# fjdf/slaMEM

Hardware: AMD Instinct MI355X
Metric: MEMs/sec (and queries/sec) on 100 Mbp ref x 10 M 150 bp queries, l=20 (higher is better)
Workload: dtype u32; 1 GPU; synthetic 100000000 bp reference (splitmix64 seed 42) x 10000000 reads/GPU of 150 bp, 2% substitutions, 50% reverse-complemented, -b -l 20; ref_len=100000000, reads_total=10000000, read_len=150, min_len=20, both_strands=True, parallelism=query shards x1, one GPU, no replication

## Files before the change

include/slamem_hip.h:

```cpp
#ifndef SLAMEM_HIP_H
#define SLAMEM_HIP_H

#include <stddef.h>
#include <stdint.h>

#ifdef __cplusplus
extern "C" {
#endif

#define SLAMEM_ABI_VERSION 4

enum {
    SLAMEM_OK = 0,
    SLAMEM_ERR_ARG = 1,
    SLAMEM_ERR_HIP = 2,
    SLAMEM_ERR_NOMEM = 3,
    SLAMEM_ERR_CAPACITY = 4,
    SLAMEM_ERR_FORMAT = 5,
    SLAMEM_ERR_IO = 6,
    SLAMEM_ERR_NO_DEVICE = 7
};

typedef struct slamem_index slamem_index;

// ... 87 lines not shown
    uint64_t skips;
    uint64_t enum_row_steps;
    uint64_t enum_levels;
    uint64_t enum_wave_us;
    uint64_t state_lane_trips[11];
    uint64_t state_wave_trips[11];
    uint64_t seed_windows;
    uint64_t seed_compares;
    uint64_t seed_letter_masks;
    uint64_t seed_mems;
    uint64_t seed_strands_left;
    uint64_t seed_reads;
    uint64_t seed_query_bytes;
    uint64_t seed_left_why[7];
    uint64_t seed_once_reads;
} slamem_search_stats;

int slamem_abi_version(void);
const char *slamem_strerror(int code);
const char *slamem_last_error_message(void);
int slamem_device_count(int *count_out);
int slamem_device_warmup(int device);
int slamem_device_pci_bus_id(int device, char *out, int out_bytes);
int slamem_device_mem_info(int device, uint64_t *free_out, uint64_t *total_out);
int slamem_get_timings(slamem_timings *out);
int slamem_reset_timings(void);
int slamem_search_stats_enable(int on);
int slamem_get_search_stats(slamem_search_stats *out);
int slamem_get_search_clock(double *us_to_empty_list, double *us_tail, double *us_wave_sum);

// ... 289 lines not shown
```

slamem_amd/capi.py:

```python
from __future__ import annotations

import ctypes as C
import os

_HERE = os.path.dirname(os.path.abspath(__file__))
LIB_PATH = os.environ.get("SLAMEM_HIP_LIB") or os.path.join(_HERE, "csrc", "libslamem_hip.so")
SYNTH_PATH = os.path.join(_HERE, "csrc", "libslamem_synth.so")

SLAMEM_OK = 0
SLAMEM_ERR_ARG = 1
SLAMEM_ERR_HIP = 2
SLAMEM_ERR_NOMEM = 3
SLAMEM_ERR_CAPACITY = 4
SLAMEM_ERR_FORMAT = 5
SLAMEM_ERR_IO = 6
SLAMEM_ERR_NO_DEVICE = 7

ARRAY_SA, ARRAY_BWT, ARRAY_LCP, ARRAY_PSV, ARRAY_NSV = range(5)
LAYOUT_AUTO, LAYOUT_FULL, LAYOUT_COMPACT = 0, 1, 2

ABI_SYMBOLS = (
    "slamem_abi_version", "slamem_strerror", "slamem_last_error_message", "slamem_device_count",
    "slamem_get_timings", "slamem_reset_timings", "slamem_device_warmup", "slamem_device_pci_bus_id",
    "slamem_index_build", "slamem_index_build_device", "slamem_index_build_layout", "slamem_index_build_device_layout",
# ... 62 lines not shown
                ("k8_ms_sum", C.c_double), ("seed_ms", C.c_float), ("mum_filter_ms", C.c_float), ("seed_ms_sum", C.c_double)]

    def as_dict(self):
        return {k: getattr(self, k) for k, _ in self._fields_}


class SearchStats(C.Structure):
    _fields_ = [(k, C.c_uint64) for k in (
        "fm_lines_top", "fm_lines_bottom", "rec_lines_fail", "rec_lines_pend", "rec_lines_flush", "query_loads",
        "lane_trips", "wave_trips", "positions", "enum_jobs", "prefilter_probes", "prefilter_query_loads",
        "prefilter_items", "items", "survivors", "mems", "overflow_records", "valid", "dir_sa_lines", "dir_group_loads",
        "dir_rec_lines", "dir_letters", "jump_lines", "skip_group_loads", "skip_probe_lines", "skip_attempts", "skips",
        "enum_row_steps", "enum_levels", "enum_wave_us")] + [("state_lane_trips", C.c_uint64 * 11),
                                                               ("state_wave_trips", C.c_uint64 * 11)] + [
        (k, C.c_uint64) for k in ("seed_windows", "seed_compares", "seed_letter_masks", "seed_mems", "seed_strands_left",
                                  "seed_reads", "seed_query_bytes")] + [("seed_left_why", C.c_uint64 * 7), ("seed_once_reads", C.c_uint64)]

    def as_dict(self):
        return {k: (list(getattr(self, k)) if (k.startswith("state_") or k == "seed_left_why") else int(getattr(self, k))) for k, _ in self._fields_}


_LIB = None
_SYNTH = None


class GtParams(C.Structure):
    _fields_ = [("ploidy", C.c_uint32), ("match_cost", C.c_uint32), ("het_cost", C.c_uint32), ("err_cost", C.c_uint32),
                ("het_prior", C.c_uint32), ("min_depth", C.c_uint32), ("min_qual", C.c_uint32)]


def _declare(L):
# ... 177 lines not shown
```

slamem_amd/csrc/mem_search.hip:

```cpp
#include "common.h"
#include "prims.h"

#include <atomic>
#include <type_traits>
#include <new>
#include <stdlib.h>
#include <string.h>

namespace slamem {

struct Blk {
    uint4 a;
    uint4 b;
    uint4 c;
    uint4 d;
};

__device__ __forceinline__ uint64_t u64_of(uint32_t lo, uint32_t hi) { return ((uint64_t)hi << 32) | lo; }

__device__ __forceinline__ Blk load_blk(const FMBlock* __restrict__ fm, uint32_t bi) {
    const uint4* p = reinterpret_cast<const uint4*>(fm + bi);
    Blk k;
    k.a = p[0]; k.b = p[1]; k.c = p[2]; k.d = p[3];
    return k;
// ... 120 lines not shown
    uint64_t num_items;
    uint8_t* item_attempt;
    const uint8_t* item_alive;
    const uint32_t* work_ids;
    const uint32_t* work_count;
    unsigned long long* stats;
    uint64_t query_words;
    const uint64_t* pq;
    uint64_t* pq_out;
    uint32_t implicit_items;
    uint32_t* seed_left_ids;
    unsigned int* seed_left_count;
    unsigned int* seed_long_flag;
    unsigned int* seed_wide;
    uint32_t seed_step;
    const uint64_t* item_pk;
    unsigned int* work_cursor;
    int32_t direct_min_depth;
    uint32_t use_jump;
    uint32_t pad2;
    uint32_t skip_w;
    const uint64_t* pq2;
    uint64_t* pq2_out;
    uint8_t* item_flags;
    uint32_t skip_s1;
    uint32_t pad4;
    const struct SliceState* slice_state;
    const uint32_t* item_block;
    struct OutCtx {
        struct RawRow* inline_rows;
// ... 806 lines not shown
        const uint2 e = A.defer.list[i];
        uint32_t* c = A.defer.pool + e.y;
        const uint32_t jobs = c[0], own = c[1];
        uint32_t run = 0;
        for (uint32_t s2 = 0; s2 < jobs; s2++) { const uint32_t v = c[2u + s2]; c[2u + s2] = run; run += v; }
        c[2u + jobs] = run;
        A.block_counts[e.x] = own + run;
    }
}

enum : uint32_t {
    SC_FM_TOP = 0, SC_FM_BOT, SC_REC_FAIL_LINES, SC_REC_PEND_LINES, SC_REC_FLUSH_LINES, SC_QUERY_LOADS, SC_LANE_TRIPS,
    SC_WAVE_TRIPS, SC_POSITIONS, SC_ENUM_JOBS, SC_ENUM_ROW_STEPS, SC_PF_PROBES, SC_PF_QUERY_LOADS, SC_PF_ITEMS,
    SC_DIR_SA, SC_DIR_GROUPS, SC_DIR_RECS, SC_DIR_QLOADS, SC_DIR_LETTERS, SC_JUMP_LINES,
    SC_SKIP_GROUPS, SC_SKIP_QLOADS, SC_SKIP_PROBES, SC_SKIP_OK, SC_T_FIRST, SC_T_DRAIN, SC_T_LAST, SC_T_WAVE_SUM, SC_ENUM_LEVELS, SC_T_ENUM_SUM, SC_STATE_TRIPS , SC_STATE_WAVES = SC_STATE_TRIPS + 11 ,
    SC_SEED_WINDOWS = SC_STATE_WAVES + 11, SC_SEED_COMPARES, SC_SEED_NMASKS, SC_SEED_MEMS, SC_SEED_LEFT, SC_SEED_READS, SC_SEED_QBYTES, SC_SEED_WHY , SC_SEED_ONCE = SC_SEED_WHY + 7, SC_COUNT
};
template <bool kStats>
__device__ __forceinline__ void stat_flush(unsigned long long* dst, uint32_t v) {
    if (!kStats) return;
    for (int o = 32; o > 0; o >>= 1) v += __shfl_down(v, o);
    if ((threadIdx.x & 63u) == 0u && v) atomicAdd(dst, (unsigned long long)v);
}

template <uint32_t kLanes>
__global__ void __launch_bounds__(256) k_pack_queries(SearchArgs A, bool long_only) {
    __shared__ uint8_t lut[512];
    for (uint32_t i = threadIdx.x; i < 256u; i += 256u) {
        uint32_t c = ascii_code_q(i);
        lut[i] = (uint8_t)c;
        lut[256u + i] = (uint8_t)(c >= 2u ? 7u - c : c);
// ... 1051 lines not shown
        const uint32_t g = list[i];
        const ItemDesc d = item_of(A, g);
        uint32_t n_probe = 0, n_qload = 0;
        if (!prefilter_item<false>(A, d, n_probe, n_qload)) alive[g] = 0;
    }
}

#ifndef SLAMEM_SEED_READS
#define SLAMEM_SEED_READS 21
#endif
constexpr uint32_t kSeedReads = SLAMEM_SEED_READS, kSeedReadsMid = 16, kSeedReadsLong = 16;
constexpr uint32_t kSeedMaxLen = 192;
constexpr uint32_t kSeedMaxLenMid = 256;
constexpr uint32_t kSeedMaxLenLong = 384;
#ifndef SLAMEM_SEED_JOBS
#define SLAMEM_SEED_JOBS 16
#endif
constexpr uint32_t kSeedJobs = SLAMEM_SEED_JOBS;
#ifndef SLAMEM_SEED_MEMS
#define SLAMEM_SEED_MEMS 12
#endif
constexpr uint32_t kSeedMems = SLAMEM_SEED_MEMS;
constexpr uint32_t kSigLetters = 12, kSigMask = (1u << kSigLetters) - 1u, kSigKnown = 1u << 24;

template <uint32_t NW, uint32_t R>
struct SeedWave {
    static constexpr uint32_t kJobs = kSeedJobs * R * NW / 3u, kMems = kSeedMems * R * NW / 3u;
    uint64_t pl[R][2][2][NW + 1];
    uint32_t len[R];
    uint32_t nwin[R];
    union {
        uint4 raw[R * NW * 4 + 1];
        struct {
            uint32_t job_p[kJobs], job_x[kJobs];
            uint32_t mem_key[kMems], mem_ref[kMems];
            uint32_t mem_sig[kMems];
        };
    };
    uint32_t bad[R];
    uint64_t pn[R][NW + 1];
    uint32_t hasn;
    unsigned long long expl[R];
    union {
        uint16_t ring[128];
        unsigned long long smask[2 * R];
    };
    uint32_t flags;
    uint32_t pad[3];
};

__device__ __forceinline__ void wave_sync() {
    __builtin_amdgcn_fence(__ATOMIC_RELEASE, "wavefront");
    __builtin_amdgcn_wave_barrier();
    __builtin_amdgcn_fence(__ATOMIC_ACQUIRE, "wavefront");
}
__device__ __forceinline__ uint64_t funnel64(uint64_t lo, uint64_t hi, uint32_t sh) { return (lo >> sh) | ((hi << 1) << (63u - sh)); }
__device__ __forceinline__ uint64_t bits_below(int x) {
    const int c = x < 0 ? 0 : x > 64 ? 64 : x;
    return c == 0 ? 0ull : (~0ull >> (64 - c));
}
__device__ __forceinline__ uint64_t bits_range(int lo, int hi) { return bits_below(hi) & ~bits_below(lo); }
__device__ __forceinline__ uint32_t sel4(const uint4& v, uint32_t a) {
    const uint32_t lo = (a & 1u) ? v.y : v.x, hi = (a & 1u) ? v.w : v.z;
    return (a & 2u) ? hi : lo;
// ... 2 lines not shown
    const uint32_t a = e & 3u, x0 = sel4(b0, a), x1 = sel4(b1, a), x2 = sel4(b2, a);
    return e < 4u ? x0 : e < 8u ? x1 : x2;
}
__device__ __forceinline__ uint32_t byte_tops(uint32_t m) {
    const uint32_t y = m >> 7;
    return (y | (y >> 7) | (y >> 14) | (y >> 21)) & 0xFu;
}

#ifndef SLAMEM_SEED_WAVES
#define SLAMEM_SEED_WAVES 1
#endif
template <bool kStats, uint32_t NW, uint32_t R>
__global__ void __launch_bounds__(256, SLAMEM_SEED_WAVES) k_seed_mems(SearchArgs A, uint8_t* __restrict__ alive) {
    constexpr uint32_t kMaxLen = 64u * NW;
    static_assert(R <= 32u && R * NW <= 128u, "a flag word holds a bit per read; the planes step runs in at most two passes");
    __shared__ SeedWave<NW, R> lds[4];
    const IndexView& ix = A.ix;
    const uint32_t lane = threadIdx.x & 63u, wv = threadIdx.x >> 6;
    SeedWave<NW, R>& S = lds[wv];
    const uint32_t strands = A.strands, k = ix.seed_k, L = A.min_len, s = L - k + 1u;
    const uint32_t kmask = (1u << k) - 1u;
    const uint64_t r0 = ((uint64_t)blockIdx.x * 4u + wv) * R;
    if (r0 >= (uint64_t)A.num_queries) return;
    const uint32_t nr = (uint64_t)A.num_queries - r0 < R ? (uint32_t)((uint64_t)A.num_queries - r0) : R;
    const unsigned long long below = (1ull << lane) - 1ull;
    const int64_t ulast = (int64_t)text_units(ix.n) - 1;
    uint32_t n_win = 0, n_cmp = 0, n_nm = 0, n_mem = 0;

    const uint64_t off = lane <= nr ? A.offsets[r0 + lane] : 0ull;
    constexpr uint32_t kRawChunks = R * NW * 4u + 1u, kSpecIters = (kRawChunks + 63u) / 64u;
// ... 142 lines not shown
                const uint64_t* f = S.pl[i][0][pl];
                const uint64_t lo = w + q < NW ? __brevll(f[NW - 1u - (w + q)]) : 0ull, hi = w + q + 1u < NW ? __brevll(f[NW - 2u - (w + q)]) : 0ull;
                S.pl[i][1][pl][w] = Li ? ~funnel64(lo, hi, r) & bits_range(0, (int)Li - 64 * (int)w) : 0ull;
            }
        }
    }
    {
        const bool isbad = lane < nr && plen != 0u && S.bad[lane] != 0u;
        wflags |= (uint32_t)__ballot(isbad);
        if (isbad) nwin = 0;
        if (lane < nr) { S.len[lane] = nwin ? len : 0u; S.nwin[lane] = nwin; }
    }
    if (lane == 0u)
        for (uint32_t i = nr; i < R; i++) { S.len[i] = 0u; S.nwin[i] = 0u; }
    wave_sync();
    const uint32_t mfit = k / s > 6u ? 6u : k / s;
    const uint32_t mstep = A.seed_step ? A.seed_step : mfit >= 3u ? mfit : s <= 12u ? 2u : 1u;

    const bool wave_hasn = __builtin_amdgcn_readfirstlane((int)S.hasn) != 0;
    uint32_t lg_slots = 0;
    {
        const uint32_t nwl = lane < nr ? S.nwin[lane] : 0u;
#pragma unroll
        for (uint32_t t = 1, lg = 1; t <= 32u; t <<= 1, lg++)
            if (__ballot(nwl > t) != 0ull) lg_slots = lg;
    }
    if (lane < R) S.expl[lane] = 0ull;
    uint32_t njobs = 0, nmems = 0;

    auto search = [&](auto with_n) {
    constexpr bool hasn = decltype(with_n)::value;
    auto trip = [&](uint32_t ent, bool act, uint32_t step) {
        const uint32_t rs = ent >> 8, wi = ent & 0xFFu;
        const uint32_t Lr = act ? S.len[rs] : 0u;
        const uint32_t o = wi * s;
        uint32_t want = 0, pal = 0;
        uint4 b0 = make_uint4(0, 0, 0, 0), b1 = b0, b2 = b0, b3 = b0;
        if (hasn && act) {
            const uint64_t* PN = S.pn[rs];
            if (((uint32_t)funnel64(PN[o >> 6], PN[(o >> 6) + 1u], o & 63u) & kmask) != 0u) act = false;
        }
        if (act) {
            const uint32_t q = o >> 6, sh = o & 63u;
            const uint64_t* P0 = S.pl[rs][0][0];
            const uint64_t* P1 = S.pl[rs][0][1];
            const uint32_t f0 = (uint32_t)funnel64(P0[q], P0[q + 1u], sh) & kmask, f1 = (uint32_t)funnel64(P1[q], P1[q + 1u], sh) & kmask;
            uint32_t bucket, tagbits, orient;
            seed_place(f0, f1, k, ix.seed_log2, bucket, tagbits, orient, pal);
            want = tagbits | (orient << 7);
            const uint4* B = reinterpret_cast<const uint4*>(ix.seed + bucket);
            b0 = B[0]; b1 = B[1]; b2 = B[2]; b3 = B[3];
        }
        if (kStats) n_win += (uint32_t)__popcll(__ballot(act));
        const uint32_t wbytes = want * 0x01010101u;
        const uint32_t x0 = b3.x ^ wbytes, x1 = b3.y ^ wbytes, x2 = b3.z ^ wbytes;
        const uint32_t m0 = ~((x0 & 0x7F7F7F7Fu) + 0x7F7F7F7Fu) & 0x80808080u, m1 = ~((x1 & 0x7F7F7F7Fu) + 0x7F7F7F7Fu) & 0x80808080u,
                       m2 = ~((x2 & 0x7F7F7F7Fu) + 0x7F7F7F7Fu) & 0x80808080u;
        const uint32_t count = b3.w;
        uint32_t hits = byte_tops(m0) | (byte_tops(m1) << 4) | (byte_tops(m2) << 8);
        const uint32_t rev = byte_tops(x0 & 0x80808080u) | (byte_tops(x1 & 0x80808080u) << 4) | (byte_tops(x2 & 0x80808080u) << 8);
        hits &= count >= kSeedSlots ? 0xFFFu : (1u << count) - 1u;
        if (strands == 1u && step == 1u) hits &= ~rev;
        if (!act) hits = 0;
        const uint32_t xn = act && (count & kSeedSpilled) ? (count >> 24) & 0x1Fu : 0u, xo = (count & 0xFFFFFFu) << 2;
        if (act && count > kSeedSlots && !(count & kSeedSpilled)) {
            atomicOr(&S.flags, 1u << rs);
            if (kStats) atomicAdd(A.stats + SC_SEED_WHY + 1u, 1ull);
            hits = 0;
        }
        const bool both = pal != 0u && strands == 2u;
        if (kStats && both && hits) atomicAdd(A.stats + SC_SEED_WHY + 2u, 1ull);
        const uint32_t e1 = hits ? (uint32_t)__ffs((int)hits) - 1u : 0u;
        const uint32_t p1 = sel12(b0, b1, b2, e1);
        const uint32_t st1 = (rev >> e1) & 1u;
        const uint32_t dist = step * s;
        uint32_t pn = 0, pp1 = 0, ps1 = 0;
        if (dist <= k) {
            pp1 = __shfl_up(p1, 1);
            ps1 = __shfl_up(hits ? st1 : 2u, 1);
            const uint32_t pent = __shfl_up(act ? ent : 0xFFFFFFFFu, 1);
            pn = (lane == 0u || wi < step || pent != ent - step || ps1 == 2u) ? 0u : 1u;
        }
        const uint32_t njobs0 = njobs;
        auto push = [&](bool hv, uint32_t p, uint32_t st) {
            const uint32_t w = st ? p + dist : p - dist;
            const bool job = hv && !(pn && pp1 == w && ps1 == st);
            const unsigned long long qb = __ballot(job);
            const uint32_t at = njobs + (uint32_t)__popcll(qb & below);
            if (job && at < SeedWave<NW, R>::kJobs) {
                S.job_p[at] = p;
                S.job_x[at] = (st ? Lr - k - o : o) | (st << 15) | (rs << 16);
            }
            njobs += (uint32_t)__popcll(qb);
        };
        uint32_t rem = hits;
        for (uint32_t it = 0; __ballot(rem != 0u) != 0ull; it++) {
            const bool hv = rem != 0u;
            const uint32_t e = it == 0u ? e1 : hv ? (uint32_t)__ffs((int)rem) - 1u : 0u;
            rem &= rem - 1u;
            const uint32_t p = it == 0u ? p1 : sel12(b0, b1, b2, e);
            push(hv, p, (rev >> e) & 1u);
            if (__ballot(hv && both) != 0ull) push(hv && both, p, 1u);
        }
        for (uint32_t e0 = 0; __ballot(e0 < xn) != 0ull; e0 += 4u) {
            const bool on = e0 < xn;
            uint4 v0 = make_uint4(0, 0, 0, 0), v1 = v0;
            if (on) {
                const uint4* P = reinterpret_cast<const uint4*>(ix.spill + xo + e0);
                v0 = P[0]; v1 = P[1];
            }
#pragma unroll
            for (uint32_t q = 0; q < 4u; q++) {
                const uint32_t p = q == 0u ? v0.x : q == 1u ? v0.z : q == 2u ? v1.x : v1.z;
                const uint32_t d = ((q == 0u ? v0.y : q == 1u ? v0.w : q == 2u ? v1.y : v1.w) ^ want) & 0xFFu;
                const uint32_t st = d >> 7;
                const bool hv = on && e0 + q < xn && (d & 0x7Fu) == 0u && !(strands == 1u && st && step == 1u);
                if (__ballot(hv) == 0ull) continue;
                push(hv, p, st);
                if (__ballot(hv && both) != 0ull) push(hv && both, p, 1u);
            }
        }
        if (njobs > SeedWave<NW, R>::kJobs) {
            if (act) atomicOr(&S.flags, 1u << rs);
            if (kStats && lane == 0u) atomicAdd(A.stats + SC_SEED_WHY + 3u, 1ull);
            njobs = njobs0;
        }
    };
    auto lookups = [&](uint32_t round) {
        const uint32_t step = round == 0u ? mstep : 1u;
        uint32_t cnt = 0;
        const uint32_t per = 64u >> lg_slots, wi = lane & ((1u << lg_slots) - 1u);
        const uint32_t wmod = wi - mstep * ((wi * (65536u / mstep + 1u)) >> 16);
        for (uint32_t r = 0;; r += per) {
            if (r < nr) {
                const uint32_t rr = r + (lane >> lg_slots);
                const uint32_t nw = (rr >= nr || ((S.flags >> rr) & 1u)) ? 0u : S.nwin[rr];
                const bool pred = wi < nw && (round == 0u ? wmod == 0u : wmod != 0u && ((S.expl[rr] >> wi) & 1ull) == 0ull);
                const unsigned long long pm = __ballot(pred);
                if (pred) S.ring[cnt + (uint32_t)__popcll(pm & below)] = (uint16_t)((rr << 8) | wi);
                cnt += (uint32_t)__popcll(pm);
            }
            const bool last = r >= nr;
            if (cnt >= 64u || (last && cnt != 0u)) {
                wave_sync();
                const bool act = lane < cnt;
                const uint32_t ent = act ? S.ring[lane] : 0u;
                const uint32_t over = lane + 64u < cnt ? S.ring[lane + 64u] : 0u;
                wave_sync();
                if (lane + 64u < cnt) S.ring[lane] = (uint16_t)over;
                cnt = cnt > 64u ? cnt - 64u : 0u;
                trip(ent, act, step);
            }
            if (last) break;
        }
        wave_sync();
    };

    auto compares = [&](uint32_t round) {
        const bool mark = round == 0u && mstep > 1u;
        const uint32_t ms = mstep * s;
        const uint32_t gone = S.flags;
        for (uint32_t jb = 0; jb < njobs; jb += 64u) {
            const bool listed = jb + lane < njobs;
            const uint32_t p = listed ? S.job_p[jb + lane] : 0u, xx = listed ? S.job_x[jb + lane] : 0u;
            const uint32_t os = xx & 0x7FFFu, st = (xx >> 15) & 1u, jr = xx >> 16;
            const bool has = listed && ((gone >> jr) & 1u) == 0u;
            const uint32_t Lj = S.len[jr];
            const int64_t d = (int64_t)p - (int64_t)os;
            const int64_t u0 = d >> 6;
            const uint32_t sh = (uint32_t)(d & 63);
            bool is_mem = false;
            uint32_t key = 0, ref = 0, sig = 0;
            if (has) {
                constexpr int NU = (int)NW + 1;
                int64_t ui[NU];
#pragma unroll
                for (int i = 0; i < NU; i++) { const int64_t u = u0 + i; ui[i] = u < 0 ? 0 : u > ulast ? ulast : u; }
                const uint4* T = reinterpret_cast<const uint4*>(ix.tpl);
                uint4 tu[NU], tx[NU];
#pragma unroll
                for (int i = 0; i < NU; i++) { tu[i] = T[2 * ui[i]]; tx[i] = T[2 * ui[i] + 1]; }
                uint64_t uq[NU], nu[NU];
                uint32_t anyn = 0;
#pragma unroll
                for (int i = 0; i < NU; i++) { nu[i] = u64_of(tx[i].x, tx[i].y); uq[i] = u64_of(tx[i].z, tx[i].w); anyn |= (tx[i].x | tx[i].y); }
                if (kStats && anyn) n_nm++;
                const uint64_t* R0 = S.pl[jr][st][0];
// ... 11 lines not shown
                    } else {
                        const uint32_t shn = kMaxLen - Lj, qn = shn >> 6, rn = shn & 63u;
#pragma unroll
                        for (int w = 0; w < (int)NW; w++) {
                            const uint32_t x = (uint32_t)w + qn;
                            const uint64_t lo64 = x < NW ? __brevll(PN[NW - 1u - x]) : 0ull, hi64 = x + 1u < NW ? __brevll(PN[NW - 2u - x]) : 0ull;
                            mm[w] |= funnel64(lo64, hi64, rn);
                        }
                    }
                }
                const int lo = d < 0 ? (int)(-d) : 0;
                const int64_t room = (int64_t)ix.n - d;
                const int hi = room < (int64_t)Lj ? (int)room : (int)Lj;
#pragma unroll
                for (int w = 0; w < (int)NW; w++) mm[w] |= ~bits_range(lo - 64 * w, hi - 64 * w);
                uint32_t a = 0, b = kMaxLen;
                bool broken = false;
#pragma unroll
                for (int w = 0; w < (int)NW; w++) {
                    const uint64_t lw = mm[w] & bits_range(0, (int)os - 64 * w);
                    if (lw) a = 64u * w + 64u - (uint32_t)__clzll((long long)lw);
                    if (mm[w] & bits_range((int)os - 64 * w, (int)(os + k) - 64 * w)) broken = true;
                }
#pragma unroll
                for (int w = (int)NW - 1; w >= 0; w--) {
                    const uint64_t hw = mm[w] & ~bits_range(0, (int)(os + k) - 64 * w);
                    if (hw) b = 64u * w + (uint32_t)__ffsll((unsigned long long)hw) - 1u;
                }
                const uint32_t af = st ? Lj - b : a, bf = st ? Lj - a : b, of = st ? Lj - k - os : os;
                bool owner;
                if (round == 0u) owner = !(of >= ms && of - ms >= af);
                else {
                    const uint32_t oa = (af + ms - 1u) / ms * ms;
                    owner = !(mstep > 1u && oa + k <= bf) && !(of >= s && of - s >= af);
                }
                if (broken) {
                    atomicOr(&S.flags, 1u << jr);
                    if (kStats) atomicAdd(A.stats + SC_SEED_WHY + 4u, 1ull);
                }
                else if (owner && b - a >= L && (strands == 2u || st == 0u)) {
                    is_mem = true; key = (a << 16) | (b - a); ref = (uint32_t)(d + (int64_t)a);
                    if (!anyn && b + kSigLetters <= kMaxLen && d + (int64_t)b + (int64_t)kSigLetters <= (int64_t)ix.n) {
                        const uint32_t wb = b >> 6, sb = b & 63u;
                        uint64_t l0 = 0, h0 = 0, l1 = 0, h1 = 0;
#pragma unroll
                        for (int w = 0; w < (int)NW; w++) {
                            const uint64_t t0 = funnel64(u64_of(tu[w].x, tu[w].y), u64_of(tu[w + 1].x, tu[w + 1].y), sh);
                            const uint64_t t1 = funnel64(u64_of(tu[w].z, tu[w].w), u64_of(tu[w + 1].z, tu[w + 1].w), sh);
                            if ((uint32_t)w == wb) { l0 = t0; l1 = t1; }
                            if ((uint32_t)w == wb + 1u) { h0 = t0; h1 = t1; }
                        }
                        sig = kSigKnown | ((uint32_t)funnel64(l0, h0, sb) & kSigMask) | (((uint32_t)funnel64(l1, h1, sb) & kSigMask) << kSigLetters);
                    }
                }
                if (mark && !broken && bf >= af + k) {
                    uint64_t uqs[NW];
#pragma unroll
                    for (int w = 0; w < (int)NW; w++) uqs[w] = funnel64(uq[w], uq[w + 1], sh);
                    unsigned long long done = 0ull;
                    for (uint32_t wi = (af + s - 1u) / s, wl = (bf - k) / s; wi <= wl; wi++) {
                        const uint32_t x = st ? Lj - k - wi * s : wi * s;
                        uint64_t word = 0ull;
#pragma unroll
                        for (int w = 0; w < (int)NW; w++) word = (x >> 6) == (uint32_t)w ? uqs[w] : word;
                        if ((word >> (x & 63u)) & 1ull) done |= 1ull << wi;
                    }
                    if (done) atomicOr(&S.expl[jr], done);
                }
            }
            if (kStats) {
                const uint32_t nh = (uint32_t)__popcll(__ballot(has));
                n_cmp += nh;
                if (mark && lane == 0u) atomicAdd(A.stats + SC_SEED_ONCE, (unsigned long long)nh);
            }
            const unsigned long long mb = __ballot(is_mem);
            if (is_mem) {
                const uint32_t at = nmems + (uint32_t)__popcll(mb & below);
                if (at < SeedWave<NW, R>::kMems) { S.mem_key[at] = key; S.mem_ref[at] = ref; S.mem_sig[at] = sig | ((2u * jr + st) << 25); }
                else { atomicOr(&S.flags, 1u << jr); if (kStats) atomicAdd(A.stats + SC_SEED_WHY + 5u, 1ull); }
            }
            nmems += (uint32_t)__popcll(mb);
        }
        wave_sync();
    };

    for (uint32_t round = 0; round < (mstep > 1u ? 2u : 1u); round++) {
        njobs = 0;
        lookups(round);
        compares(round);
    }
    };
    if (wave_hasn) search(std::true_type{}); else search(std::false_type{});
    {
        if (nmems > SeedWave<NW, R>::kMems) nmems = SeedWave<NW, R>::kMems;

        const uint32_t g0 = (uint32_t)(r0 * strands);
        auto rank_of = [&](uint32_t mi, uint32_t key, uint32_t g, uint32_t& rank, uint32_t& cnt, bool& tie) {
            rank = 0; cnt = 0; tie = false;
            for (uint32_t t2 = 0; t2 < nmems; t2++) {
                const uint32_t kk = S.mem_key[t2], gg = S.mem_sig[t2] >> 25;
                const bool same = gg == g;
                cnt += same ? 1u : 0u;
                rank += (same && kk > key) ? 1u : 0u;
                tie = tie || (same && kk == key && t2 != mi);
// ... 90 lines not shown
        if (lane < nr * strands) alive[r0 * strands + lane] = isleft ? 1 : 0;
        const unsigned long long lm = __ballot(isleft);
        if (lm != 0ull) {
            unsigned int at = 0;
            if (lane == 0u) at = atomicAdd(A.seed_left_count, (unsigned int)__popcll(lm));
            at = (unsigned int)__builtin_amdgcn_readfirstlane((int)at);
            if (isleft) A.seed_left_ids[at + (uint32_t)__popcll(lm & below)] = (uint32_t)(r0 * strands + lane);
        }
    }
    if (kStats) {
        stat_flush<kStats>(A.stats + SC_SEED_NMASKS, n_nm);
        stat_flush<kStats>(A.stats + SC_SEED_MEMS, n_mem);
        if (lane == 0u) {
            atomicAdd(A.stats + SC_SEED_WINDOWS, (unsigned long long)n_win);
            atomicAdd(A.stats + SC_SEED_COMPARES, (unsigned long long)n_cmp);
            atomicAdd(A.stats + SC_SEED_READS, (unsigned long long)nr);
            atomicAdd(A.stats + SC_SEED_QBYTES, (unsigned long long)(__builtin_amdgcn_readlane((int)(uint32_t)off, (int)nr) - __builtin_amdgcn_readlane((int)(uint32_t)off, 0)));
            atomicAdd(A.stats + SC_SEED_LEFT, (unsigned long long)(strands * (uint32_t)__popc(fl)));
            atomicAdd(A.stats + SC_SEED_WHY + 0u, (unsigned long long)__popc(wflags));
        }
    }
}

__global__ void __launch_bounds__(256) k_place_inline(const RawRow* __restrict__ inl, uint64_t stride, const uint32_t* __restrict__ counts,
                                                      const uint64_t* __restrict__ item_off, uint64_t nitems,
                                                      const uint32_t* __restrict__ sa, uint64_t capacity,
                                                      slamem_mem* __restrict__ out, const uint8_t* __restrict__ inline_valid) {
    uint64_t g = (uint64_t)blockIdx.x * blockDim.x + threadIdx.x;
    if (g >= nitems) return;
    uint32_t cnt = counts[g];
// ... 532 lines not shown
    (void)hipEventRecord(ev[0], stream);
    if (nitems && (match_type != 1 || mam_v3)) {
        static const bool use_filter = [] { const char* v = getenv("SLAMEM_KFILTER"); return !(v && atoi(v) == 0); }();
        seeded = seed_path;
        if (seeded) {
            uint8_t* d_alive = reinterpret_cast<uint8_t*>(ws + w.off_alive);
            if (mems_capacity && !A.skip_w && !want_stats && enum_chunks()) {
                STEP(hipMemsetAsync(ws + w.off_rawkey, 0xFF, mems_capacity * sizeof(RawKey), stream), "memset");
                rawkey_marked = true;
            }
            STEP(hipMemsetAsync(d_counts, 0, nitems * 4, stream), "memset");
            STEP(hipMemsetAsync(A.item_attempt, 0, nitems, stream), "memset");
            {
                const char* v = getenv("SLAMEM_SEED_STEP");
                A.seed_step = v && atoi(v) >= 1 && atoi(v) <= 6 ? (uint32_t)atoi(v) : 0u;
            }
            uint32_t* d_ids = reinterpret_cast<uint32_t*>(ws + w.off_workids);
            uint32_t* d_nwork = reinterpret_cast<uint32_t*>(d_total) + 8;
            A.seed_left_ids = d_ids;
            A.seed_left_count = d_nwork;
            A.seed_long_flag = reinterpret_cast<unsigned int*>(d_total) + 3;
            A.seed_wide = reinterpret_cast<unsigned int*>(d_total) + 4;
            seed_words_avg = query_bytes > (uint64_t)num_queries * kSeedMaxLenMid ? 6u : query_bytes > (uint64_t)num_queries * kSeedMaxLen ? 4u : 3u;
            const uint32_t hint = __atomic_load_n(&idx->seed_words_hint, __ATOMIC_RELAXED);
            seed_words = seed_words_avg > hint ? seed_words_avg : hint;
            const bool mid_reads = seed_words == 4u, long_reads = seed_words == 6u;
            const dim3 gs(grid_for((uint64_t)num_queries, 4 * (long_reads ? kSeedReadsLong : mid_reads ? kSeedReadsMid : kSeedReads)));
            if (long_reads) {
                if (want_stats) hipLaunchKernelGGL((k_seed_mems<true, 6, kSeedReadsLong>), gs, dim3(256), 0, stream, A, d_alive);
                else hipLaunchKernelGGL((k_seed_mems<false, 6, kSeedReadsLong>), gs, dim3(256), 0, stream, A, d_alive);
// ... 352 lines not shown
        o.dir_letters = c[SC_DIR_LETTERS]; o.jump_lines = c[SC_JUMP_LINES];
        o.skip_group_loads = c[SC_SKIP_GROUPS]; o.skip_probe_lines = c[SC_SKIP_PROBES]; o.skips = c[SC_SKIP_OK];
        o.skip_attempts = c[SC_SKIP_QLOADS];
        o.enum_row_steps = c[SC_ENUM_ROW_STEPS]; o.enum_levels = c[SC_ENUM_LEVELS];
        last_search_clock()[0] = (c[SC_T_DRAIN] - c[SC_T_FIRST]) / 100.0;
        last_search_clock()[1] = (c[SC_T_LAST] - c[SC_T_DRAIN]) / 100.0;
        last_search_clock()[2] = c[SC_T_WAVE_SUM] / 100.0;
        o.enum_wave_us = c[SC_T_ENUM_SUM] / 100;
        for (int q = 0; q < 11; q++) { o.state_lane_trips[q] = c[SC_STATE_TRIPS + q]; o.state_wave_trips[q] = c[SC_STATE_WAVES + q]; }
        o.prefilter_probes = c[SC_PF_PROBES]; o.prefilter_query_loads = c[SC_PF_QUERY_LOADS]; o.prefilter_items = c[SC_PF_ITEMS];
        o.seed_windows = c[SC_SEED_WINDOWS]; o.seed_compares = c[SC_SEED_COMPARES]; o.seed_letter_masks = c[SC_SEED_NMASKS];
        o.seed_mems = c[SC_SEED_MEMS]; o.seed_strands_left = c[SC_SEED_LEFT]; o.seed_reads = c[SC_SEED_READS];
        o.seed_query_bytes = c[SC_SEED_QBYTES];
        for (int q = 0; q < 7; q++) o.seed_left_why[q] = c[SC_SEED_WHY + q];
        o.seed_once_reads = c[SC_SEED_ONCE];
        o.items = nitems;
        o.survivors = prefiltered ? nwork : nitems;
        o.mems = total;
        o.overflow_records = listed;
        o.valid = match_type != 1 ? 1 : 0;
    }
    float ms = 0, ms_prep = 0, ms_k8 = 0;
    if (hipEventElapsedTime(&ms, ev[0], ev[5]) == hipSuccess) ms_prep = ms;
    if (timed_k8 && hipEventElapsedTime(&ms, ev[4], ev[1]) == hipSuccess) {
        ms_k8 = ms;
        tm.t.k8_ms = ms;
        tm.t.k8_ms_sum += ms;
    } else if (hipEventElapsedTime(&ms, ev[5], ev[1]) == hipSuccess) ms_k8 = ms;
    tm.t.search_kernel_ms = ms_prep + ms_k8;
    tm.t.search_kernel_ms_sum += ms_prep + ms_k8;
// ... 157 lines not shown
```

Baseline: 4.499 billion MEMs/s.

## Seed MEMs from a few probe windows with per-read diagonal dedup chains

Replaces the fixed-stride first-round window sampling with a small number of evenly spaced probe windows per read (default three, tunable via an environment variable). Jobs are keyed by diagonal and chained per read so that compares on an already-seen diagonal are dropped. Each compare now enumerates every maximal run on its diagonal, rather than only the run around the seed, and marks all windows that run covers as explored. The aim is fewer k-mer lookups and fewer redundant compares per read, at the cost of chain walks in LDS, a heavier per-job bit-run enumeration, and retuned job and MEM capacities that risk more overflow fallbacks.

```diff
diff --git a/include/slamem_hip.h b/include/slamem_hip.h
--- a/include/slamem_hip.h
+++ b/include/slamem_hip.h
@@ -125,6 +125,7 @@
     uint64_t seed_query_bytes;
     uint64_t seed_left_why[7];
     uint64_t seed_once_reads;
+    uint64_t seed_dropped_same_diagonal;
 } slamem_search_stats;
 
 int slamem_abi_version(void);
diff --git a/slamem_amd/capi.py b/slamem_amd/capi.py
--- a/slamem_amd/capi.py
+++ b/slamem_amd/capi.py
@@ -100,7 +100,8 @@
         "enum_row_steps", "enum_levels", "enum_wave_us")] + [("state_lane_trips", C.c_uint64 * 11),
                                                                ("state_wave_trips", C.c_uint64 * 11)] + [
         (k, C.c_uint64) for k in ("seed_windows", "seed_compares", "seed_letter_masks", "seed_mems", "seed_strands_left",
-                                  "seed_reads", "seed_query_bytes")] + [("seed_left_why", C.c_uint64 * 7), ("seed_once_reads", C.c_uint64)]
+                                  "seed_reads", "seed_query_bytes")] + [("seed_left_why", C.c_uint64 * 7), ("seed_once_reads", C.c_uint64),
+                                                                                              ("seed_dropped_same_diagonal", C.c_uint64)]
 
     def as_dict(self):
         return {k: (list(getattr(self, k)) if (k.startswith("state_") or k == "seed_left_why") else int(getattr(self, k))) for k, _ in self._fields_}
diff --git a/slamem_amd/csrc/mem_search.hip b/slamem_amd/csrc/mem_search.hip
--- a/slamem_amd/csrc/mem_search.hip
+++ b/slamem_amd/csrc/mem_search.hip
@@ -158,6 +158,7 @@
     unsigned int* seed_long_flag;
     unsigned int* seed_wide;
     uint32_t seed_step;
+    uint32_t seed_probes;
     const uint64_t* item_pk;
     unsigned int* work_cursor;
     int32_t direct_min_depth;
@@ -994,7 +995,7 @@
     SC_WAVE_TRIPS, SC_POSITIONS, SC_ENUM_JOBS, SC_ENUM_ROW_STEPS, SC_PF_PROBES, SC_PF_QUERY_LOADS, SC_PF_ITEMS,
     SC_DIR_SA, SC_DIR_GROUPS, SC_DIR_RECS, SC_DIR_QLOADS, SC_DIR_LETTERS, SC_JUMP_LINES,
     SC_SKIP_GROUPS, SC_SKIP_QLOADS, SC_SKIP_PROBES, SC_SKIP_OK, SC_T_FIRST, SC_T_DRAIN, SC_T_LAST, SC_T_WAVE_SUM, SC_ENUM_LEVELS, SC_T_ENUM_SUM, SC_STATE_TRIPS , SC_STATE_WAVES = SC_STATE_TRIPS + 11 ,
-    SC_SEED_WINDOWS = SC_STATE_WAVES + 11, SC_SEED_COMPARES, SC_SEED_NMASKS, SC_SEED_MEMS, SC_SEED_LEFT, SC_SEED_READS, SC_SEED_QBYTES, SC_SEED_WHY , SC_SEED_ONCE = SC_SEED_WHY + 7, SC_COUNT
+    SC_SEED_WINDOWS = SC_STATE_WAVES + 11, SC_SEED_COMPARES, SC_SEED_NMASKS, SC_SEED_MEMS, SC_SEED_LEFT, SC_SEED_READS, SC_SEED_QBYTES, SC_SEED_WHY , SC_SEED_ONCE = SC_SEED_WHY + 7, SC_SEED_DROPPED, SC_COUNT
 };
 template <bool kStats>
 __device__ __forceinline__ void stat_flush(unsigned long long* dst, uint32_t v) {
@@ -2076,11 +2077,11 @@
 constexpr uint32_t kSeedMaxLenMid = 256;
 constexpr uint32_t kSeedMaxLenLong = 384;
 #ifndef SLAMEM_SEED_JOBS
-#define SLAMEM_SEED_JOBS 16
+#define SLAMEM_SEED_JOBS 22
 #endif
 constexpr uint32_t kSeedJobs = SLAMEM_SEED_JOBS;
 #ifndef SLAMEM_SEED_MEMS
-#define SLAMEM_SEED_MEMS 12
+#define SLAMEM_SEED_MEMS 8
 #endif
 constexpr uint32_t kSeedMems = SLAMEM_SEED_MEMS;
 constexpr uint32_t kSigLetters = 12, kSigMask = (1u << kSigLetters) - 1u, kSigKnown = 1u << 24;
@@ -2108,8 +2109,10 @@
         unsigned long long smask[2 * R];
     };
     uint32_t flags;
-    uint32_t pad[3];
+    uint32_t nmem;
+    uint32_t head[R];
 };
+constexpr uint32_t kNoJob = 0xFFFFu, kJobKey = 0xFE00u;
 
 __device__ __forceinline__ void wave_sync() {
     __builtin_amdgcn_fence(__ATOMIC_RELEASE, "wavefront");
@@ -2142,6 +2145,7 @@
 __global__ void __launch_bounds__(256, SLAMEM_SEED_WAVES) k_seed_mems(SearchArgs A, uint8_t* __restrict__ alive) {
     constexpr uint32_t kMaxLen = 64u * NW;
     static_assert(R <= 32u && R * NW <= 128u, "a flag word holds a bit per read; the planes step runs in at most two passes");
+    static_assert(NW != 3u || sizeof(SeedWave<NW, R>) * 4u <= 40u * 1024u, "four blocks a CU in the form for reads of up to 192 letters");
     __shared__ SeedWave<NW, R> lds[4];
     const IndexView& ix = A.ix;
     const uint32_t lane = threadIdx.x & 63u, wv = threadIdx.x >> 6;
@@ -2314,8 +2318,18 @@
     if (lane == 0u)
         for (uint32_t i = nr; i < R; i++) { S.len[i] = 0u; S.nwin[i] = 0u; }
     wave_sync();
+    constexpr uint32_t kProbes = 3u;
     const uint32_t mfit = k / s > 6u ? 6u : k / s;
-    const uint32_t mstep = A.seed_step ? A.seed_step : mfit >= 3u ? mfit : s <= 12u ? 2u : 1u;
+    const uint32_t mstep = A.seed_step ? A.seed_step : (A.seed_probes || mfit >= 3u || s <= 12u) ? 0u : 1u;
+    const uint32_t nprobe = mstep ? 0u : A.seed_probes ? A.seed_probes : kProbes;
+    const uint32_t nrounds = mstep == 1u ? 1u : 2u;
+    const uint32_t pdiv = 65536u / (2u * (nprobe ? nprobe : 1u)) + 1u;
+    uint64_t sper = 0ull;
+    for (uint32_t x = 0; x < 64u; x += s) sper |= 1ull << x;
+    const uint32_t smagic = s > 1u ? (uint32_t)(0xFFFFFFFFu / s) + 1u : 0u;
+    uint32_t smod[NW];
+#pragma unroll
+    for (uint32_t w = 0; w < NW; w++) smod[w] = (64u * w) % s;
 
     const bool wave_hasn = __builtin_amdgcn_readfirstlane((int)S.hasn) != 0;
     uint32_t lg_slots = 0;
@@ -2325,12 +2339,22 @@
         for (uint32_t t = 1, lg = 1; t <= 32u; t <<= 1, lg++)
             if (__ballot(nwl > t) != 0ull) lg_slots = lg;
     }
-    if (lane < R) S.expl[lane] = 0ull;
-    uint32_t njobs = 0, nmems = 0;
+    if (lane < R) {
+        unsigned long long pm = 0ull;
+        if (mstep) for (uint32_t x = 0; x < 64u; x += mstep) pm |= 1ull << x;
+        else {
+            const uint32_t nw = lane < nr ? S.nwin[lane] : 0u;
+            for (uint32_t j = 0; j < nprobe; j++) pm |= 1ull << (((2u * j + 1u) * nw * pdiv) >> 16);
+        }
+        S.expl[lane] = pm;
+        S.head[lane] = kNoJob;
+    }
+    if (lane == 0u) S.nmem = 0u;
+    uint32_t njobs = 0, nmems = 0, n_drop = 0;
 
     auto search = [&](auto with_n) {
     constexpr bool hasn = decltype(with_n)::value;
-    auto trip = [&](uint32_t ent, bool act, uint32_t step) {
+    auto trip = [&](uint32_t ent, bool act, bool last) {
         const uint32_t rs = ent >> 8, wi = ent & 0xFFu;
         const uint32_t Lr = act ? S.len[rs] : 0u;
         const uint32_t o = wi * s;
@@ -2360,7 +2384,7 @@
         uint32_t hits = byte_tops(m0) | (byte_tops(m1) << 4) | (byte_tops(m2) << 8);
         const uint32_t rev = byte_tops(x0 & 0x80808080u) | (byte_tops(x1 & 0x80808080u) << 4) | (byte_tops(x2 & 0x80808080u) << 8);
         hits &= count >= kSeedSlots ? 0xFFFu : (1u << count) - 1u;
-        if (strands == 1u && step == 1u) hits &= ~rev;
+        if (strands == 1u && last) hits &= ~rev;
         if (!act) hits = 0;
         const uint32_t xn = act && (count & kSeedSpilled) ? (count >> 24) & 0x1Fu : 0u, xo = (count & 0xFFFFFFu) << 2;
         if (act && count > kSeedSlots && !(count & kSeedSpilled)) {
@@ -2373,24 +2397,21 @@
         const uint32_t e1 = hits ? (uint32_t)__ffs((int)hits) - 1u : 0u;
         const uint32_t p1 = sel12(b0, b1, b2, e1);
         const uint32_t st1 = (rev >> e1) & 1u;
-        const uint32_t dist = step * s;
-        uint32_t pn = 0, pp1 = 0, ps1 = 0;
-        if (dist <= k) {
-            pp1 = __shfl_up(p1, 1);
-            ps1 = __shfl_up(hits ? st1 : 2u, 1);
-            const uint32_t pent = __shfl_up(act ? ent : 0xFFFFFFFFu, 1);
-            pn = (lane == 0u || wi < step || pent != ent - step || ps1 == 2u) ? 0u : 1u;
-        }
-        const uint32_t njobs0 = njobs;
+        const uint32_t pp1 = __shfl_up(p1, 1), ps1 = __shfl_up(hits ? st1 : 2u, 1);
+        const uint32_t pent = __shfl_up(act ? ent : 0xFFFFFFFFu, 1);
+        const bool pn = lane != 0u && (pent >> 8) == rs && ps1 != 2u;
+        const uint32_t dist = (wi - (pent & 0xFFu)) * s;
         auto push = [&](bool hv, uint32_t p, uint32_t st) {
             const uint32_t w = st ? p + dist : p - dist;
             const bool job = hv && !(pn && pp1 == w && ps1 == st);
+            if (kStats) n_drop += (uint32_t)__popcll(__ballot(hv && !job));
             const unsigned long long qb = __ballot(job);
             const uint32_t at = njobs + (uint32_t)__popcll(qb & below);
             if (job && at < SeedWave<NW, R>::kJobs) {
-                S.job_p[at] = p;
-                S.job_x[at] = (st ? Lr - k - o : o) | (st << 15) | (rs << 16);
-            }
+                const uint32_t os = st ? Lr - k - o : o;
+                S.job_p[at] = p - os;
+                S.job_x[at] = os | ((p < os ? 1u : 0u) << 9) | (st << 10) | (rs << 11) | (atomicExch(&S.head[rs], at) << 16);
+            } else if (job) atomicOr(&S.flags, 1u << rs);
             njobs += (uint32_t)__popcll(qb);
         };
         uint32_t rem = hits;
@@ -2414,34 +2435,32 @@
                 const uint32_t p = q == 0u ? v0.x : q == 1u ? v0.z : q == 2u ? v1.x : v1.z;
                 const uint32_t d = ((q == 0u ? v0.y : q == 1u ? v0.w : q == 2u ? v1.y : v1.w) ^ want) & 0xFFu;
                 const uint32_t st = d >> 7;
-                const bool hv = on && e0 + q < xn && (d & 0x7Fu) == 0u && !(strands == 1u && st && step == 1u);
+                const bool hv = on && e0 + q < xn && (d & 0x7Fu) == 0u && !(strands == 1u && st && last);
                 if (__ballot(hv) == 0ull) continue;
                 push(hv, p, st);
                 if (__ballot(hv && both) != 0ull) push(hv && both, p, 1u);
             }
         }
         if (njobs > SeedWave<NW, R>::kJobs) {
-            if (act) atomicOr(&S.flags, 1u << rs);
             if (kStats && lane == 0u) atomicAdd(A.stats + SC_SEED_WHY + 3u, 1ull);
-            njobs = njobs0;
+            njobs = SeedWave<NW, R>::kJobs;
         }
     };
     auto lookups = [&](uint32_t round) {
-        const uint32_t step = round == 0u ? mstep : 1u;
+        const bool last = round + 1u == nrounds;
         uint32_t cnt = 0;
         const uint32_t per = 64u >> lg_slots, wi = lane & ((1u << lg_slots) - 1u);
-        const uint32_t wmod = wi - mstep * ((wi * (65536u / mstep + 1u)) >> 16);
         for (uint32_t r = 0;; r += per) {
             if (r < nr) {
                 const uint32_t rr = r + (lane >> lg_slots);
                 const uint32_t nw = (rr >= nr || ((S.flags >> rr) & 1u)) ? 0u : S.nwin[rr];
-                const bool pred = wi < nw && (round == 0u ? wmod == 0u : wmod != 0u && ((S.expl[rr] >> wi) & 1ull) == 0ull);
+                const bool pred = wi < nw && (uint32_t)((S.expl[rr] >> wi) & 1ull) == (round == 0u ? 1u : 0u);
                 const unsigned long long pm = __ballot(pred);
                 if (pred) S.ring[cnt + (uint32_t)__popcll(pm & below)] = (uint16_t)((rr << 8) | wi);
                 cnt += (uint32_t)__popcll(pm);
             }
-            const bool last = r >= nr;
-            if (cnt >= 64u || (last && cnt != 0u)) {
+            const bool drain = r >= nr;
+            if (cnt >= 64u || (drain && cnt != 0u)) {
                 wave_sync();
                 const bool act = lane < cnt;
                 const uint32_t ent = act ? S.ring[lane] : 0u;
@@ -2449,28 +2468,40 @@
                 wave_sync();
                 if (lane + 64u < cnt) S.ring[lane] = (uint16_t)over;
                 cnt = cnt > 64u ? cnt - 64u : 0u;
-                trip(ent, act, step);
-            }
-            if (last) break;
+                trip(ent, act, last);
+            }
+            if (drain) break;
         }
         wave_sync();
     };
 
-    auto compares = [&](uint32_t round) {
-        const bool mark = round == 0u && mstep > 1u;
-        const uint32_t ms = mstep * s;
+    auto compares = [&](uint32_t round, uint32_t jfirst) {
+        const bool mark = round + 1u < nrounds;
         const uint32_t gone = S.flags;
-        for (uint32_t jb = 0; jb < njobs; jb += 64u) {
+        for (uint32_t jb = jfirst; jb < njobs; jb += 64u) {
             const bool listed = jb + lane < njobs;
-            const uint32_t p = listed ? S.job_p[jb + lane] : 0u, xx = listed ? S.job_x[jb + lane] : 0u;
-            const uint32_t os = xx & 0x7FFFu, st = (xx >> 15) & 1u, jr = xx >> 16;
-            const bool has = listed && ((gone >> jr) & 1u) == 0u;
+            const uint32_t dlo = listed ? S.job_p[jb + lane] : 0u, xx = listed ? S.job_x[jb + lane] : 0u;
+            const uint32_t os = xx & 0x1FFu, st = (xx >> 10) & 1u, jr = (xx >> 11) & 0x1Fu;
+            bool has = listed && ((gone >> jr) & 1u) == 0u;
+            if (has) {
+                uint32_t pv = xx >> 16, it = 0;
+                for (; pv != kNoJob && it < SeedWave<NW, R>::kJobs; it++) {
+                    const uint32_t qp = S.job_p[pv], qx = S.job_x[pv];
+                    if (qp == dlo && ((qx ^ xx) & kJobKey) == 0u) break;
+                    pv = qx >> 16;
+                }
+                if (pv != kNoJob) {
+                    has = false;
+                    if (it == SeedWave<NW, R>::kJobs) {
+                        atomicOr(&S.flags, 1u << jr);
+                        if (kStats) atomicAdd(A.stats + SC_SEED_WHY + 3u, 1ull);
+                    } else if (kStats) atomicAdd(A.stats + SC_SEED_DROPPED, 1ull);
+                }
+            }
             const uint32_t Lj = S.len[jr];
-            const int64_t d = (int64_t)p - (int64_t)os;
+            const int64_t d = (xx >> 9) & 1u ? (int64_t)(int32_t)dlo : (int64_t)dlo;
             const int64_t u0 = d >> 6;
             const uint32_t sh = (uint32_t)(d & 63);
-            bool is_mem = false;
-            uint32_t key = 0, ref = 0, sig = 0;
             if (has) {
                 constexpr int NU = (int)NW + 1;
                 int64_t ui[NU];
@@ -2512,32 +2543,58 @@
                 const int hi = room < (int64_t)Lj ? (int)room : (int)Lj;
 #pragma unroll
                 for (int w = 0; w < (int)NW; w++) mm[w] |= ~bits_range(lo - 64 * w, hi - 64 * w);
-                uint32_t a = 0, b = kMaxLen;
                 bool broken = false;
 #pragma unroll
+                for (int w = 0; w < (int)NW; w++)
+                    if (mm[w] & bits_range((int)os - 64 * w, (int)(os + k) - 64 * w)) broken = true;
+                uint64_t rk[NW], rl[NW];
+#pragma unroll
+                for (int w = 0; w < (int)NW; w++) rk[w] = rl[w] = ~mm[w];
+                for (uint32_t c = 1u, goal = k > 1u ? k : L; c < L;) {
+                    const uint32_t left = goal - c, t = left < c ? (left < 63u ? left : 63u) : (c < 63u ? c : 63u);
+#pragma unroll
+                    for (int w = 0; w < (int)NW; w++) rl[w] &= funnel64(rl[w], w + 1 < (int)NW ? rl[w + 1] : 0ull, t);
+                    c += t;
+                    if (c == k) {
+#pragma unroll
+                        for (int w = 0; w < (int)NW; w++) rk[w] = rl[w];
+                        goal = L;
+                    }
+                }
+                uint64_t rs0[NW];
+                uint32_t cnt = 0;
+#pragma unroll
                 for (int w = 0; w < (int)NW; w++) {
-                    const uint64_t lw = mm[w] & bits_range(0, (int)os - 64 * w);
-                    if (lw) a = 64u * w + 64u - (uint32_t)__clzll((long long)lw);
-                    if (mm[w] & bits_range((int)os - 64 * w, (int)(os + k) - 64 * w)) broken = true;
-                }
-#pragma unroll
-                for (int w = (int)NW - 1; w >= 0; w--) {
-                    const uint64_t hw = mm[w] & ~bits_range(0, (int)(os + k) - 64 * w);
-                    if (hw) b = 64u * w + (uint32_t)__ffsll((unsigned long long)hw) - 1u;
-                }
-                const uint32_t af = st ? Lj - b : a, bf = st ? Lj - a : b, of = st ? Lj - k - os : os;
-                bool owner;
-                if (round == 0u) owner = !(of >= ms && of - ms >= af);
-                else {
-                    const uint32_t oa = (af + ms - 1u) / ms * ms;
-                    owner = !(mstep > 1u && oa + k <= bf) && !(of >= s && of - s >= af);
+                    rs0[w] = rl[w] & ((mm[w] << 1) | (w ? mm[w - 1] >> 63 : 1ull));
+                    cnt += (uint32_t)__popcll(rs0[w]);
                 }
                 if (broken) {
                     atomicOr(&S.flags, 1u << jr);
                     if (kStats) atomicAdd(A.stats + SC_SEED_WHY + 4u, 1ull);
-                }
-                else if (owner && b - a >= L && (strands == 2u || st == 0u)) {
-                    is_mem = true; key = (a << 16) | (b - a); ref = (uint32_t)(d + (int64_t)a);
+                    cnt = 0;
+                }
+                if (strands == 1u && st != 0u) cnt = 0;
+                uint32_t at = cnt ? atomicAdd(&S.nmem, cnt) : 0u;
+                if (cnt && at + cnt > SeedWave<NW, R>::kMems) {
+                    atomicOr(&S.flags, 1u << jr);
+                    if (kStats) atomicAdd(A.stats + SC_SEED_WHY + 5u, 1ull);
+                    cnt = at < SeedWave<NW, R>::kMems ? SeedWave<NW, R>::kMems - at : 0u;
+                }
+                for (; cnt != 0u; cnt--, at++) {
+                    uint32_t a = 0, b = kMaxLen;
+#pragma unroll
+                    for (int w = (int)NW - 1; w >= 0; w--)
+                        if (rs0[w]) a = 64u * w + (uint32_t)__ffsll((unsigned long long)rs0[w]) - 1u;
+#pragma unroll
+                    for (int w = 0; w < (int)NW; w++)
+                        if (a >> 6 == (uint32_t)w) rs0[w] &= rs0[w] - 1ull;
+#pragma unroll
+                    for (int w = (int)NW - 1; w >= 0; w--) {
+                        const uint64_t hw = mm[w] & ~bits_range(0, (int)(a + L) - 64 * w);
+                        if (hw) b = 64u * w + (uint32_t)__ffsll((unsigned long long)hw) - 1u;
+                    }
+                    const uint32_t key = (a << 16) | (b - a), ref = (uint32_t)(d + (int64_t)a);
+                    uint32_t sig = 0;
                     if (!anyn && b + kSigLetters <= kMaxLen && d + (int64_t)b + (int64_t)kSigLetters <= (int64_t)ix.n) {
                         const uint32_t wb = b >> 6, sb = b & 63u;
                         uint64_t l0 = 0, h0 = 0, l1 = 0, h1 = 0;
@@ -2550,18 +2607,20 @@
                         }
                         sig = kSigKnown | ((uint32_t)funnel64(l0, h0, sb) & kSigMask) | (((uint32_t)funnel64(l1, h1, sb) & kSigMask) << kSigLetters);
                     }
-                }
-                if (mark && !broken && bf >= af + k) {
-                    uint64_t uqs[NW];
+                    S.mem_key[at] = key; S.mem_ref[at] = ref; S.mem_sig[at] = sig | ((2u * jr + st) << 25);
+                }
+                if (mark && !broken) {
+                    const uint32_t x0 = st ? Lj - k - (S.nwin[jr] - 1u) * s : 0u;
+                    unsigned long long done = 0ull;
 #pragma unroll
-                    for (int w = 0; w < (int)NW; w++) uqs[w] = funnel64(uq[w], uq[w + 1], sh);
-                    unsigned long long done = 0ull;
-                    for (uint32_t wi = (af + s - 1u) / s, wl = (bf - k) / s; wi <= wl; wi++) {
-                        const uint32_t x = st ? Lj - k - wi * s : wi * s;
-                        uint64_t word = 0ull;
-#pragma unroll
-                        for (int w = 0; w < (int)NW; w++) word = (x >> 6) == (uint32_t)w ? uqs[w] : word;
-                        if ((word >> (x & 63u)) & 1ull) done |= 1ull << wi;
+                    for (int w = 0; w < (int)NW; w++) {
+                        const uint32_t c = smod[w], f = x0 >= c ? x0 - c : x0 + s - c;
+                        uint64_t m = f < 64u ? rk[w] & funnel64(uq[w], uq[w + 1], sh) & (sper << f) : 0ull;
+                        for (; m != 0ull; m &= m - 1ull) {
+                            const uint32_t x = 64u * w + (uint32_t)__ffsll((unsigned long long)m) - 1u;
+                            const uint32_t of = st ? Lj - k - x : x;
+                            done |= 1ull << (s > 1u ? __umulhi(of, smagic) : of);
+                        }
                     }
                     if (done) atomicOr(&S.expl[jr], done);
                 }
@@ -2571,21 +2630,15 @@
                 n_cmp += nh;
                 if (mark && lane == 0u) atomicAdd(A.stats + SC_SEED_ONCE, (unsigned long long)nh);
             }
-            const unsigned long long mb = __ballot(is_mem);
-            if (is_mem) {
-                const uint32_t at = nmems + (uint32_t)__popcll(mb & below);
-                if (at < SeedWave<NW, R>::kMems) { S.mem_key[at] = key; S.mem_ref[at] = ref; S.mem_sig[at] = sig | ((2u * jr + st) << 25); }
-                else { atomicOr(&S.flags, 1u << jr); if (kStats) atomicAdd(A.stats + SC_SEED_WHY + 5u, 1ull); }
-            }
-            nmems += (uint32_t)__popcll(mb);
         }
         wave_sync();
+        nmems = (uint32_t)__builtin_amdgcn_readfirstlane((int)S.nmem);
     };
 
-    for (uint32_t round = 0; round < (mstep > 1u ? 2u : 1u); round++) {
-        njobs = 0;
+    for (uint32_t round = 0; round < nrounds; round++) {
+        const uint32_t jfirst = njobs;
         lookups(round);
-        compares(round);
+        compares(round, jfirst);
     }
     };
     if (wave_hasn) search(std::true_type{}); else search(std::false_type{});
@@ -2706,6 +2759,7 @@
         if (lane == 0u) {
             atomicAdd(A.stats + SC_SEED_WINDOWS, (unsigned long long)n_win);
             atomicAdd(A.stats + SC_SEED_COMPARES, (unsigned long long)n_cmp);
+            atomicAdd(A.stats + SC_SEED_DROPPED, (unsigned long long)n_drop);
             atomicAdd(A.stats + SC_SEED_READS, (unsigned long long)nr);
             atomicAdd(A.stats + SC_SEED_QBYTES, (unsigned long long)(__builtin_amdgcn_readlane((int)(uint32_t)off, (int)nr) - __builtin_amdgcn_readlane((int)(uint32_t)off, 0)));
             atomicAdd(A.stats + SC_SEED_LEFT, (unsigned long long)(strands * (uint32_t)__popc(fl)));
@@ -3268,6 +3322,8 @@
             {
                 const char* v = getenv("SLAMEM_SEED_STEP");
                 A.seed_step = v && atoi(v) >= 1 && atoi(v) <= 6 ? (uint32_t)atoi(v) : 0u;
+                const char* pr = getenv("SLAMEM_SEED_PROBES");
+                A.seed_probes = pr && atoi(pr) >= 1 && atoi(pr) <= 8 ? (uint32_t)atoi(pr) : 0u;
             }
             uint32_t* d_ids = reinterpret_cast<uint32_t*>(ws + w.off_workids);
             uint32_t* d_nwork = reinterpret_cast<uint32_t*>(d_total) + 8;
@@ -3650,6 +3706,7 @@
         o.seed_query_bytes = c[SC_SEED_QBYTES];
         for (int q = 0; q < 7; q++) o.seed_left_why[q] = c[SC_SEED_WHY + q];
         o.seed_once_reads = c[SC_SEED_ONCE];
+        o.seed_dropped_same_diagonal = c[SC_SEED_DROPPED];
         o.items = nitems;
         o.survivors = prefiltered ? nwork : nitems;
         o.mems = total;
```

Measured after the change: 5.085 billion MEMs/s, median of 6. +13.0%, better.
